# zju3dv/ENeRF

Hardware: AMD Instinct MI355X
Metric: rendered frames/sec @512x640 3-src-view (higher is better)
Workload: dtype f32

## Files before the change

### enerf_amd/csrc/capi.hip

```cpp
#include <stdarg.h>
#include <stdint.h>
#include <stdio.h>
#include <string.h>

#include "kernels.h"
#include "prep_job.h"

using namespace enerf;

namespace enerf {
__global__ __launch_bounds__(256) void k_zero(unsigned* __restrict__ p, long long n) {
    for (long long i = (long long)blockIdx.x * blockDim.x + threadIdx.x; i < n; i += (long long)gridDim.x * blockDim.x) p[i] = 0u;
}
void zero_async(void* p, size_t bytes, hipStream_t st) {
    const long long n = (long long)(bytes / 4);
    if (n <= 0) return;
    long long blocks = cdivl(n, 256 * 4);
    if (blocks > 4096) blocks = 4096;
    ENERF_LAUNCH_SIMPLE(k_zero, (unsigned)blocks, 256, 0, st, (unsigned*)p, n);
}
void zero_async2(void* p, size_t bytes_p, void* q, size_t bytes_q, hipStream_t st) {
    if ((char*)p + bytes_p == (char*)q && bytes_p % 4 == 0) { zero_async(p, bytes_p + bytes_q, st); return; }
    zero_async(p, bytes_p, st);
    zero_async(q, bytes_q, st);
// ... 194 lines not shown
        if (im.pk8 >= 0) launch_conv3d_pk8_pack(w, wd, s.cin, p + im.pk8, st);
        if (im.b4 >= 0) launch_conv3d_b4_pack(w, wd, s.cin, p + im.b4, st);
        p += im.floats;
    }
    return check_launch("cost_reg_pack");
}
size_t enerf_cost_reg_workspace_bytes(int full, int B, int D, int h, int w) {
    long long floats[kNumBufs], f = 0;
    const int n = costreg_buffers(full, (long long)B * D * h * w, floats);
    for (int i = 0; i < n; ++i) f += floats[i];
    return (size_t)f * sizeof(float);
}
int enerf_cost_reg(const float* packed, int in_channels, int full, const float* vol, int B, int D, int h, int w,
                   float* feat, float* prob, void* workspace, size_t workspace_bytes, const enerf_options_t* options,
                   enerf_stream_t stream) {
    return cost_reg_run(packed, in_channels, full, vol, 0, B, D, h, w, feat, prob, workspace, workspace_bytes, options,
                        (hipStream_t)stream);
}
}
namespace enerf {
bool cost_reg_conv0_planar(const enerf_options_t& o, int in_channels, int full, int B, int D, int h, int w) {
    return cost_reg_plan(in_channels, full, B, D, h, w, o, device_cu_count()).vol_planar_ok;
}
int cost_reg_run(const float* packed, int in_channels, int full, const float* vol, int vol_planar, int B, int D, int h, int w,
                 float* feat, float* prob, void* workspace, size_t workspace_bytes, const enerf_options_t* options,
                 hipStream_t st, const CostRegHook* hook) {
    REQUIRE(packed && vol && feat && prob && workspace, "cost_reg: null pointer");
    REQUIRE(in_channels == 8 || in_channels == 16 || in_channels == 32, "cost_reg: in_channels=%d unsupported (8/16/32)",
            in_channels);
    REQUIRE(B > 0 && D > 0 && h > 0 && w > 0, "cost_reg: bad shape");
    int div = full ? 8 : 4;
    REQUIRE(D % div == 0 && h % div == 0 && w % div == 0, "cost_reg: D,h,w (%d,%d,%d) must be divisible by %d", D, h, w, div);
    if (workspace_bytes < enerf_cost_reg_workspace_bytes(full, B, D, h, w))
        return fail(ENERF_EWORKSPACE, "cost_reg: workspace too small");
    const CostRegPlan P = cost_reg_plan(in_channels, full, B, D, h, w, resolve_options(options), device_cu_count());
    if (vol_planar && !P.vol_planar_ok)
        return fail(ENERF_EINVAL, "cost_reg: a quad-planar volume needs the asynchronously staged conv0 kernel (conv3d_b4 0/2, D % 4 == 0, >= conv3d_lds_min_voxels)");
    float* buf[kNumBufs] = {};
    long long floats[kNumBufs];
    const int nbuf = costreg_buffers(full, (long long)B * D * h * w, floats);
    float* ws = (float*)workspace;
    for (int i = 0; i < nbuf; ++i) { buf[i] = ws; ws += floats[i]; }
    bool ok = true;
    const float* p = packed;
    for (int i = 0; i < P.n; ++i) {
        const LayerSpec& s = P.spec[i];
        const Conv3dImage im = layer_image(s);
        Conv3dDesc d = conv3d_desc(p, im, s.cin, s.cout, s.kind, s.relu);
        p += im.floats;
        d.in_planar = i == 0 ? vol_planar : (i == P.n - 1 && P.heads_planar);
// ... 624 lines not shown
```

### enerf_amd/csrc/conv3d.hip

```cpp

#include "kernels.h"

namespace enerf {

__host__ __device__ __forceinline__ void convt_axis(int par, int idx, int& k, int& dq) {
    if (par == 0) { k = 1; dq = 0; }
    else if (idx == 0) { k = 0; dq = 1; }
    else { k = 2; dq = 0; }
}
__host__ __device__ __forceinline__ int convt_class_ntaps(int cls) {
    return (1 + ((cls >> 2) & 1)) * (1 + ((cls >> 1) & 1)) * (1 + (cls & 1));
}
__host__ __device__ __forceinline__ int convt_class_offset(int cls) {
    int o = 0;
    for (int c = 0; c < cls; ++c) o += convt_class_ntaps(c);
    return o;
}

__host__ __device__ __forceinline__ int conv_cpl(int cin) { return cin >= 16 ? 4 : cin / 4; }

long long conv3d_packed_floats(int cin, int cout, int kind) {
    (void)kind;
    int rt = cdiv(cout, 16);
    return 27LL * (cin / 4) * rt * 64;
// ... 591 lines not shown
                   o.conv3d_lds_min_voxels > 0 ? o.conv3d_lds_min_voxels : 16384, vox_in, n_out, cdiv(L.cout, 16)};
    Conv3dRoute r;
    if ((r = route_t2_all(g)).family) return r;
    if ((r = route_t2_lds(g)).family) return r;
    if ((r = route_s2_lds(g)).family) return r;
    if ((r = route_b4(g)).family) return r;
    if ((r = route_pk8(g)).family) return r;
    if ((r = route_s1_lds(g)).family) return r;
    bool small;
    const Conv3dRoute global = route_global(g, &small);
    if ((r = route_wl(g, global, small)).family) return r;
    return global;
}
bool conv3d_route_planar_in(const Conv3dRoute& r) { return r.family == kRouteB4g || r.family == kRouteB4c; }
bool conv3d_route_planar_out(const Conv3dRoute& r) { return r.family == kRouteT2All && r.cout == 8; }
void conv3d_route_name(const Conv3dRoute& r, char* buf, size_t cap) {
    const char* tf = r.heads ? "true" : "false";
    switch (r.family) {
        case kRouteT2All: snprintf(buf, cap, "t2_all<%d,%d,%d,%d>", r.cin, r.cout, r.bd, r.bh); break;
        case kRouteT2Lds: snprintf(buf, cap, "t2_lds<%d>", r.cin); break;
        case kRouteS2Lds: snprintf(buf, cap, "s2_lds<%d>", r.cin); break;
        case kRouteB4: snprintf(buf, cap, "s1_b4<%d,%d,%s>", r.cin, r.bd, tf); break;
        case kRouteB4g: snprintf(buf, cap, "s1_b4g<%d,%d,%s>", r.cin, r.bd, tf); break;
        case kRouteB4c: snprintf(buf, cap, "s1_b4c<%d,%d,%s>", r.cin, r.bd, tf); break;
        case kRoutePk8: snprintf(buf, cap, "s1_pk8<%d,%d>", r.cin, r.bd); break;
        case kRouteS1Lds: snprintf(buf, cap, "s1_lds<%d,%d,%d,%d>", r.cin, r.rt, r.bd, r.bh); break;
        case kRouteWl: snprintf(buf, cap, "wl<%d,%d,%d>", r.cin, r.kind, r.ctb); break;
        case kRouteGlobal: snprintf(buf, cap, "conv3d<%d,%d,%d,%d,%d>", r.cin, r.rt, r.kind, r.ct, r.split); break;
        default: snprintf(buf, cap, "none"); break;
    }
// ... 69 lines not shown
```

### enerf_amd/csrc/conv3d_b4.hip

```cpp
#include "kernels.h"

namespace enerf {

#define ENERF_MFMA4(a, b, c) __builtin_amdgcn_mfma_f32_4x4x1f32((a), (b), (c), 0, 0, 0)

constexpr int kB4cRegs = 14;
long long conv3d_b4_packed_floats(int cin) { return 27LL * (cin / 4) * 48 + (long long)(cin / 4) * kB4cRegs * 64; }

__global__ __launch_bounds__(256) void k_conv3d_b4_pack(const float* __restrict__ w, const float* __restrict__ wd, int cin,
                                                        float* __restrict__ packed) {
    const long long total = 27LL * (cin / 4) * 48;
    const long long idx = (long long)blockIdx.x * blockDim.x + threadIdx.x;
    if (idx >= total) {
        const long long k = idx - total;
        if (k >= (long long)(cin / 4) * kB4cRegs * 64) return;
        const int l = (int)(k & 63), rr = (int)((k >> 6) % kB4cRegs), cq = (int)((k >> 6) / kB4cRegs), c = rr * 16 + (l >> 2);
        const int half = c & 1, ch = (c >> 1) & 3, tap = c >> 3;
        packed[idx] = tap < 27 ? w[((long long)(4 * half + (l & 3)) * cin + 4 * cq + ch) * 27 + tap] : 0.f;
        return;
    }
    const int e = (int)(idx % 48), r = e & 3, i = (e >> 2) & 3, slot = e >> 4;
    const long long q = idx / 48;
    const int nq = cin / 4, cq = (int)(q % nq), tap = (int)(q / nq);
    if (slot < 2) packed[idx] = w[((long long)(4 * slot + i) * cin + 4 * cq + r) * 27 + tap];
// ... 29 lines not shown
    int t = (int)xcd_contiguous(blockIdx.x, gridDim.x);
    const int bw = t % nbw; t /= nbw;
    const int bh = t % nbh; t /= nbh;
    const int bd = t % nbd;
    const int b = t / nbd;
    const int x0 = bw * BW, y0 = bh * BH, z0 = bd * BD;

    f32x4 acc[V][2];
    float dacc[V];
#pragma unroll
    for (int v = 0; v < V; ++v) { acc[v][0] = f32x4{0.f, 0.f, 0.f, 0.f}; acc[v][1] = f32x4{0.f, 0.f, 0.f, 0.f}; dacc[v] = 0.f; }
    const float* inb = in + (long long)b * D * H * W * CIN;
    const float* lbase = lds + ((zl * HY + yl) * HX + xl) * 4;
    const float* wbase = wlds + li * 4;

#pragma unroll 1
    for (int cb = 0; cb < NCB; ++cb) {
        if (cb > 0) __syncthreads();
        {
            constexpr int RW = HX * QV, SLOTS = 256 / RW, NR = HZ * HY, NITR = (NR + SLOTS - 1) / SLOTS;
            const int sub = tid % RW, slot = tid / RW, sdx = sub / QV, sq = sub - sdx * QV;
            const int gx = x0 + sdx - 1;
            const bool colok = slot < SLOTS && gx >= 0 && gx < W;
            float4 sv[NITR], wq[NWIT];
            bool sk[NITR];
            const float* src = inb + cb * CB + sq * 4;
#pragma unroll
            for (int it = 0; it < NITR; ++it) {
                const int r = slot + it * SLOTS, dz = r / HY, dy = r - dz * HY;
                const int gy = y0 + dy - 1, gz = z0 + dz - 1;
// ... 47 lines not shown
            if (HEADS) {
#pragma unroll
                for (int q = 0; q < QV; ++q)
#pragma unroll
                    for (int v = 0; v < V; ++v) {
                        const float4 bb = bq[tap & 1][v][q], wd = aq[tap & 1][q][NS - 1];
                        dacc[v] = __builtin_fmaf(wd.x, bb.x, dacc[v]);
                        dacc[v] = __builtin_fmaf(wd.y, bb.y, dacc[v]);
                        dacc[v] = __builtin_fmaf(wd.z, bb.z, dacc[v]);
                        dacc[v] = __builtin_fmaf(wd.w, bb.w, dacc[v]);
                        ENERF_PIN_VGPR(dacc[v]);
                    }
            }
#pragma unroll
            for (int q = 0; q < QV; ++q) {
                const float4 A0 = aq[tap & 1][q][0], A1 = aq[tap & 1][q][1];
                const float a0[4] = {A0.x, A0.y, A0.z, A0.w}, a1[4] = {A1.x, A1.y, A1.z, A1.w};
#pragma unroll
                for (int r = 0; r < 4; ++r)
#pragma unroll
                    for (int v = 0; v < V; ++v) {
                        const float4 bb = bq[tap & 1][v][q];
                        const float bx = r == 0 ? bb.x : r == 1 ? bb.y : r == 2 ? bb.z : bb.w;
                        acc[v][0] = ENERF_MFMA4(a0[r], bx, acc[v][0]);
                        acc[v][1] = ENERF_MFMA4(a1[r], bx, acc[v][1]);
                    }
            }
            __builtin_amdgcn_sched_barrier(0);
        }
    }

    const int x = x0 + xl, y = y0 + yl;
    if (x >= W || y >= H) return;
#pragma unroll
    for (int v = 0; v < V; ++v) {
        const int z = z0 + zl + 2 * v;
        if (z >= D) continue;
        const long long o = (((long long)b * D + z) * H + y) * W + x;
#pragma unroll
        for (int half = 0; half < 2; ++half) {
            float yv[4];
#pragma unroll
            for (int r = 0; r < 4; ++r) {
                yv[r] = acc[v][half][r] * scale[4 * half + r] + shift[4 * half + r];
                if (relu) yv[r] = fmaxf(yv[r], 0.f);
            }
            *reinterpret_cast<float4*>(out + o * 8 + 4 * half) = make_float4(yv[0], yv[1], yv[2], yv[3]);
        }
        if (HEADS && out2 != nullptr) out2[o] = dacc[v] * scale[8] + shift[8];
    }
}

__device__ float g_b4_zeros[64];

template <int CIN, int BD, bool HEADS>
__global__ __launch_bounds__(256, 3) void k_conv3d_s1_b4g(const float* __restrict__ wb4, const float* __restrict__ scale,
                                                          const float* __restrict__ shift, const float* __restrict__ in,
                                                          float* __restrict__ out, float* __restrict__ out2, int relu, int B,
                                                          int D, int H, int W, int nbd, int nbh, int nbw, int in_planar) {
    constexpr int BH = 8, BW = 16, V = BD / 2;
    constexpr int NQ = CIN / 4, NS = HEADS ? 3 : 2;
    constexpr int HX = BW + 2, HY = BH + 2, HZ = BD + 2, NVOX = HZ * HY * HX;
    constexpr int NCH = (NVOX + 63) / 64, PLANE = NCH * 64 * 4;
    constexpr int NW4 = 27 * NS * 4, NWCH = (NW4 + 63) / 64;
    constexpr int BUF = PLANE + NWCH * 64 * 4;
    constexpr int MYCH = (NCH + 3) / 4, MYW = (NWCH + 3) / 4;
    ENERF_DYN_SMEM(float, lds);

    const int tid = threadIdx.x, li = tid & 3, lane = tid & 63;
    const int wv = __builtin_amdgcn_readfirstlane(tid >> 6);
    const int m = lane & 31;
    const bool g1 = (m >= 4 && m < 12) || (m >= 16 && m < 20) || m >= 28;
    const int xl = g1 ? (m < 12 ? m - 4 : m < 20 ? m - 8 : m - 16) : (m < 4 ? m : m < 16 ? m - 8 : m - 12);
    const int yl = 4 * (wv & 1) + 2 * (lane >> 5) + (g1 ? 1 : 0), zl = wv >> 1;
// ... 104 lines not shown
            for (int r = 0; r < 4; ++r) {
                yv[r] = acc[v][half][r] * scale[4 * half + r] + shift[4 * half + r];
                if (relu) yv[r] = fmaxf(yv[r], 0.f);
            }
            *reinterpret_cast<float4*>(out + o * 8 + 4 * half) = make_float4(yv[0], yv[1], yv[2], yv[3]);
        }
        if (HEADS && out2 != nullptr) out2[o] = dacc[v] * scale[8] + shift[8];
    }
}

template <int CIN, int BD, bool HEADS>
__global__ __launch_bounds__(256, 3) void k_conv3d_s1_b4c(const float* __restrict__ wb4, const float* __restrict__ scale,
                                                          const float* __restrict__ shift, const float* __restrict__ in,
                                                          float* __restrict__ out, float* __restrict__ out2, int relu, int B,
                                                          int D, int H, int W, int nbd, int nbh, int nbw, int in_planar) {
    constexpr int BH = 8, BW = 16, V = BD / 2;
    constexpr int NQ = CIN / 4;
    constexpr int HX = BW + 2, HY = BH + 2, HZ = BD + 2, NVOX = HZ * HY * HX;
    constexpr int NCH = (NVOX + 63) / 64, PLANE = NCH * 64 * 4;
    constexpr int BUF = PLANE + (HEADS ? 256 : 0);
    constexpr int MYCH = (NCH + 3) / 4;
    static_assert(NQ % 2 == 0, "passes are processed in pairs (two register sets)");
    ENERF_DYN_SMEM(float, lds);

    const int tid = threadIdx.x, lane = tid & 63;
    const int wv = __builtin_amdgcn_readfirstlane(tid >> 6);
    const int m = lane & 31;
    const bool g1 = (m >= 4 && m < 12) || (m >= 16 && m < 20) || m >= 28;
    const int xl = g1 ? (m < 12 ? m - 4 : m < 20 ? m - 8 : m - 16) : (m < 4 ? m : m < 16 ? m - 8 : m - 12);
    const int yl = 4 * (wv & 1) + 2 * (lane >> 5) + (g1 ? 1 : 0), zl = wv >> 1;
// ... 162 lines not shown
```

### enerf_amd/csrc/frame.hip

```cpp
#include <stdint.h>
#include <string.h>

#include "kernels.h"
#include "prep_job.h"
#include "side_lane.h"

using namespace enerf;

namespace enerf {

constexpr int kMaskPerThread = 4;
constexpr int kMaskPerBlock = 256 * kMaskPerThread;

__device__ __forceinline__ bool mask_set(const unsigned char* m, int eb, long long i, long long n) {
    if (i >= n) return false;
    if (eb == 1) return m[i] != 0;
    const unsigned char* p = m + i * eb;
    unsigned v = 0;
    for (int k = 0; k < eb; ++k) v |= p[k];
    return v != 0;
}
__device__ __forceinline__ int block_exclusive_scan(int v, int* sh, int& total) {
    const int t = threadIdx.x;
    sh[t] = v;
// ... 129 lines not shown
}
int check_render_feat(const char* who, const enerf_cascade_t& c, int i, const FeatDims& fd, int Hr, int Wr, bool same_extent) {
    const int fl = c.render_im_feat_level[i];
    REQUIRE(fl >= 0 && fl <= 2 && fd.c[fl] == c.nerf_model_feat_ch[i],
            "%s: render_im_feat_level[%d]=%d does not have nerf_model_feat_ch=%d channels", who, i, fl, c.nerf_model_feat_ch[i]);
    if (same_extent)
        REQUIRE(fd.h[fl] == Hr && fd.w[fl] == Wr, "%s: level %d renders at %dx%d but feature level_%d is %dx%d "
                "(the HIP FeatureNet path needs render_scale == im_ibr_scale)", who, i, Hr, Wr, fl, fd.h[fl], fd.w[fl]);
    return ENERF_OK;
}

struct LevelPlan {
    int D, h, w, C, Hs, Ws;
    int Hr, Wr, render, masked, F, Ns;
    int fl, from_l2;
    long long n_rays;
    size_t proj, dv, nf, vol, feat3d, prob, depth, std, dmvs, tex, rays;
};
struct FramePlan {
    int tex2, hip_feats, cached;
    size_t f[3], featnet_ws, featnet_ws_bytes, costreg_ws, costreg_ws_bytes;
    size_t cam_exts, cam_ixts;
    size_t ray_index, ray_count, mask_ws;
    LevelPlan L[ENERF_MAX_LEVELS];
    size_t total_floats;
};

int make_plan(const enerf_frame_args_t* a, FramePlan* P, bool cached = false) {
    REQUIRE(a, "forward: null args");
    const enerf_cascade_t& c = a->cas;
// ... 27 lines not shown
        L.D = c.volume_planes[i];
        L.h = scaled(a->H, c.volume_scale[i]);
        L.w = scaled(a->W, c.volume_scale[i]);
        REQUIRE(i < 3, "forward: level %d has no feature map (FeatureNet has three scales)", i);
        L.C = fd.c[i]; L.Hs = fd.h[i]; L.Ws = fd.w[i];
        REQUIRE(!(i == 2 && P->tex2), "forward: level_2 texels cannot feed a cost volume");
        REQUIRE(L.D > 0 && L.h > 0 && L.w > 0, "forward: level %d volume is empty", i);
        if (i > 0) REQUIRE(c.depth_inv[i - 1], "forward: cascade levels after a depth-space level are undefined in the "
                                               "reference (utils.py:130)");
        REQUIRE(a->cost_reg_packed[i], "forward: cost_reg_packed[%d] missing", i);
        const long long nv = (long long)a->B * L.D * L.h * L.w;
        L.proj = take((size_t)a->B * a->S * 12);
        L.dv = take((size_t)nv);
        L.nf = take((size_t)a->B * 2 * L.h * L.w);
        L.vol = take((size_t)nv * L.C);
        L.feat3d = take((size_t)nv * 8);
        L.prob = take((size_t)nv);
        L.depth = take((size_t)a->B * L.h * L.w);
        L.std = take((size_t)a->B * L.h * L.w);
        L.dmvs = take((size_t)a->B * L.h * L.w);
        const size_t cw = enerf_cost_reg_workspace_bytes(i != 0, a->B, L.D, L.h, L.w);
        if (cw > P->costreg_ws_bytes) P->costreg_ws_bytes = cw;
        L.render = c.render_if[i] != 0;
        if (!L.render) continue;
        L.Hr = scaled(a->H, c.render_scale[i]);
        L.Wr = scaled(a->W, c.render_scale[i]);
        L.Ns = c.num_samples[i];
        L.F = c.nerf_model_feat_ch[i] + 3;
        REQUIRE(L.Hr > 1 && L.Wr > 1, "forward: level %d render extent too small", i);
        REQUIRE(a->nerf_packed[i], "forward: nerf_packed[%d] missing", i);
        REQUIRE(a->rgb[i] && a->depth[i] && a->weights[i] && a->depth_mvs[i] && a->std[i], "forward: level %d output missing", i);
// ... 287 lines not shown
            launch_feature_volume(f[i], proj, dv, a->B, a->S, L.C, L.Hs, L.Ws, L.D, L.h, L.w, vol, st, 1);
            rc = check_launch("build_feature_volume");
        }
        if (rc == ENERF_OK) mark(ENERF_STAGE_LEVEL(i, ENERF_STAGE_VOLUME));
        return rc;
    }

    int level_cost_reg(int i) {
        const LevelPlan& L = P.L[i];
        const CostRegHook hook = {[](void* self) { static_cast<FrameRun*>(self)->enqueue_stage2(); }, this, gate_mode == 4 ? 2 : 0};
        const CostRegHook* hk = nullptr;
        const bool gated_here = !stage2_enqueued && i == cas().num - 1;
        if (gated_here) {
            if (gate_mode == 3) enqueue_stage2(); else hk = &hook;
        }
        int rc = cost_reg_run(a->cost_reg_packed[i], L.C, i != 0, ws + L.vol, vol_planar, a->B, L.D, L.h, L.w, ws + L.feat3d, ws + L.prob,
                              ws + P.costreg_ws, P.costreg_ws_bytes, a->options, st, hk);
        if (gated_here) enqueue_stage2();
        if (rc == ENERF_OK && stage2_rc != ENERF_OK) rc = stage2_rc;
        if (rc == ENERF_OK) mark(ENERF_STAGE_LEVEL(i, ENERF_STAGE_COST_REG));
        return rc;
    }

    int level_depth(int i) {
        const enerf_cascade_t& c = cas();
        const LevelPlan& L = P.L[i];
        float *prob = ws + L.prob, *dv = ws + L.dv, *depth = ws + L.depth, *std = std_of(i);
        const bool defer_regression = !L.render && i + 1 < c.num && !(a->options && a->options->fuse_depth_prep == 1);
        if (defer_regression) { pending_prob = prob; pending_dv = dv; pending_D = L.D; pending_inv = c.depth_inv[i]; }
        else launch_depth_regression(prob, dv, a->B, L.D, L.h, L.w, c.depth_inv[i], depth, std, L.render ? a->depth_mvs[i] : nullptr, st);
        mark(ENERF_STAGE_LEVEL(i, ENERF_STAGE_DEPTH_REG));
        pdepth = depth; pstd = std; pnf = ws + L.nf; hp = L.h; wp = L.w;
// ... 695 lines not shown
```

### enerf_amd/csrc/kernels.h

```cpp
#pragma once
#include "common.h"
#include "../../include/enerf_hip.h"

namespace enerf {

using Options = enerf_options_t;
inline Options resolve_options(const enerf_options_t* o) { return o ? *o : Options{}; }
int fail(int code, const char* fmt, ...);
int check_launch(const char* what);
const char* last_error();
#define REQUIRE(cond, ...) \
    do { if (!(cond)) return ::enerf::fail(ENERF_EINVAL, __VA_ARGS__); } while (0)
int device_cu_count();
void zero_async(void* p, size_t bytes, hipStream_t st);
void zero_async2(void* p, size_t bytes_p, void* q, size_t bytes_q, hipStream_t st);

void launch_channels_last(const float* src, float* dst, int n, int C, long long P, int Cpad, hipStream_t st);
void launch_channels_first(const float* src, float* dst, int n, int C, long long P, int Cpad, hipStream_t st);
void launch_pack_img_feat_rgb(const float* im_feat, int C, int Hf, int Wf, const float* src_inps, int H, int W,
                              int Hr, int Wr, int tex, int n_img, float* out, hipStream_t st);
void launch_proj_mats(const float* src_ixts, const float* src_exts, const float* tar_ixt, const float* tar_ext, int B,
                      int S, float src_scale, float tar_scale, float* proj, hipStream_t st);
void launch_depth_values(const float* near_far, const float* pdepth, const float* pstd, const float* pnf, int B, int D,
                         int h, int w, int hp, int wp, int depth_inv, float* dv, float* nf_out, hipStream_t st);
// ... 1 lines not shown
                       float src_scale, float tar_scale, float* proj, const float* near_far, const float* pdepth,
                       const float* pstd, const float* pnf, int B, int D, int h, int w, int hp, int wp, int depth_inv,
                       float* dv, float* nf_out, hipStream_t st);
void launch_depth_regression(const float* prob, const float* dv, int B, int D, int h, int w, int depth_inv,
                             float* depth, float* std, float* depth_mvs, hipStream_t st);
bool launch_regress_and_values(const float* src_ixts, const float* src_exts, const float* tar_ixt, const float* tar_ext, int S,
                               float src_scale, float tar_scale, float* proj, const float* prob_p, const float* dv_p,
                               const float* nf_p, int Dp, int hp, int wp, int depth_inv_p, float* depth_p, float* std_p, int B,
                               int D, int h, int w, int depth_inv, float* dv, float* nf_out, hipStream_t st);
void launch_build_rays(const float* rays8, const float* depth, const float* std, const float* nf, int B, int N, int h,
                       int w, int Hr, int Wr, int depth_inv, float* rays12, hipStream_t st);

void launch_feature_volume(const float* feat_nhwc, const float* proj, const float* dv, int B, int S, int C, int Hs,
                           int Ws, int D, int h, int w, float* vol, hipStream_t st, int planar = 0);
bool cost_reg_conv0_planar(const enerf_options_t& o, int in_channels, int full, int B, int D, int h, int w);
struct CostRegHook { void (*fn)(void* ctx); void* ctx; int after_layer; };
int cost_reg_run(const float* packed, int in_channels, int full, const float* vol, int vol_planar, int B, int D, int h, int w,
                 float* feat, float* prob, void* workspace, size_t workspace_bytes, const enerf_options_t* options, hipStream_t st,
                 const CostRegHook* hook = nullptr);

enum ConvKind { kConvS1 = 0, kConvS2 = 1, kConvT2 = 2 };
struct Conv3dDesc {
    const float* w;
    const float* scale;
    const float* shift;
    int cin, cout, kind, relu;
    const float* w_pk8;
    const float* w_b4;
    const float* w_t2pair;
    int in_planar;
// ... 20 lines not shown
    kRouteGlobal
};
struct Conv3dRoute {
    int family = kRouteNone;
    int cin = 0, cout = 0, kind = 0;
    int bd = 0, bh = 0;
    bool heads = false;
    int rt = 0, ct = 0, split = 0;
    int ctb = 0, kdlo = 0, nkd = 0;
};
struct Conv3dLayer { int cin, cout, kind; bool pk8, b4, t2pair; };
Conv3dRoute conv3d_route(const Conv3dLayer& L, bool has_residual, bool has_out2, int B, int Di, int Hi, int Wi, const Options& o,
                         int cu_count);
bool conv3d_route_planar_in(const Conv3dRoute& r);
bool conv3d_route_planar_out(const Conv3dRoute& r);
void conv3d_route_name(const Conv3dRoute& r, char* buf, size_t cap);

void launch_conv3d_b4(const Conv3dDesc& L, const Conv3dRoute& r, const float* in, float* out, float* out2, int B, int D, int H, int W,
                      hipStream_t st);
void launch_conv3d_pk8(const Conv3dDesc& L, const Conv3dRoute& r, const float* in, float* out, float* out2, int B, int D, int H, int W,
                       hipStream_t st);
void launch_conv3d_s2_lds(const Conv3dDesc& L, const float* in, float* out, int B, int Di, int Hi, int Wi, hipStream_t st);
void launch_conv3d_t2_lds(const Conv3dDesc& L, const float* in, const float* residual, float* out, int B, int Di, int Hi, int Wi,
                          hipStream_t st);
void launch_conv3d_t2_all(const Conv3dDesc& L, const Conv3dRoute& r, const float* in, const float* residual, float* out, int B, int Di,
                          int Hi, int Wi, hipStream_t st);
bool launch_conv3d_wl(const Conv3dDesc& L, const Conv3dRoute& r, const float* in, float* out, int B, int Di, int Hi, int Wi,
                      hipStream_t st);
long long conv3d_packed_floats(int cin, int cout, int kind);
void launch_conv3d_pack(const float* w, const float* w2, int cout1, const float* bn_w, const float* bn_b, const float* bn_mean, const float* bn_var,
// ... 134 lines not shown
```

### enerf_amd/lib.py

```python
from __future__ import annotations

import contextlib
import ctypes as C
import os
import threading
from typing import Optional

import torch

_PKG = os.path.dirname(os.path.abspath(__file__))
LIB_PATH = os.path.join(_PKG, "libenerf_hip.so")
ABI_VERSION = 11

_f = C.c_void_p
_i = C.c_int
_ll = C.c_longlong
_fl = C.c_float


class ConvBn(C.Structure):
    _fields_ = [("w", _f), ("bn_weight", _f), ("bn_bias", _f), ("bn_mean", _f), ("bn_var", _f)]


class CostRegRaw(C.Structure):
# ... 2 lines not shown

class FeatNetRaw(C.Structure):
    _fields_ = [("conv", ConvBn * 6)] + [(n, _f) for n in ("toplayer_w", "toplayer_b", "lat1_w", "lat1_b", "lat0_w",
                                                            "lat0_b", "smooth1_w", "smooth1_b", "smooth0_w", "smooth0_b")]


class NerfRaw(C.Structure):
    _fields_ = [(n, _f) for n in ("view_w", "view_b", "glob_w", "glob_b", "aggw_w", "aggw_b", "fc_w", "fc_b",
                                  "lr0_w", "lr0_b", "sigma_w", "sigma_b", "col0_w", "col0_b", "col2_w", "col2_b")]


class Options(C.Structure):
    _fields_ = [("conv3d_global_only", _i), ("conv3d_lds_min_voxels", _ll), ("conv3d_pk8", _i),
                ("featnet_unfused", _i), ("featnet_smooth0_plain", _i), ("conv3d_b4", _i), ("single_stream", _i),
                ("side_gate", _i), ("fuse_depth_prep", _i), ("conv3d_t2_variant", _i), ("conv3d_small_variant", _i),
                ("render_precision", _i)]

    def __repr__(self):
        return "Options(" + ", ".join(f"{n}={getattr(self, n)}" for n, _ in self._fields_ if getattr(self, n)) + ")"


def throughput_options() -> "Options":
    return Options(single_stream=1)


def _opt(o):
    return None if o is None else C.byref(o)


class MlpBwdArgs(C.Structure):
    _fields_ = ([(n, _f) for n in ("vox", "x", "g_raw", "packed", "bimg", "g_vox", "g_x")] + [("save", C.c_void_p * 16),
# ... 142 lines not shown
    "enerf_pack_img_feat_rgb": (_i, [_f, _i, _i, _i, _f, _i, _i, _i, _i, _i, _i, _f, _f]),
    "enerf_feature_net_packed_floats": (_ll, []),
    "enerf_feature_net_pack": (_i, [C.POINTER(FeatNetRaw), _f, _f]),
    "enerf_feature_net_workspace_bytes": (C.c_size_t, [_i, _i, _i]),
    "enerf_feature_net": (_i, [_f, _f, _i, _i, _i, _f, _f, _f, _i, _f, C.c_size_t, C.POINTER(Options), _f]),
    "enerf_feature_net_stage": (_i, [_f, _f, _i, _i, _i, _f, _f, _f, _i, _f, C.c_size_t, _i, C.POINTER(Options), _f]),
    "enerf_pack_texels_cl": (_i, [_f, _i, _f, _i, _i, _i, _i, _i, _i, _f, _f]),
    "enerf_get_proj_mats": (_i, [_f, _f, _f, _f, _i, _i, _fl, _fl, _f, _f]),
    "enerf_get_depth_values": (_i, [_f, _f, _f, _f, _i, _i, _i, _i, _i, _i, _i, _f, _f, _f]),
    "enerf_level_prep": (_i, [_f, _f, _f, _f, _i, _i, _fl, _fl, _f, _f, _f, _f, _f, _i, _i, _i, _i, _i, _i, _f, _f, _f]),
    "enerf_build_feature_volume": (_i, [_f, _f, _f, _i, _i, _i, _i, _i, _i, _i, _i, _f, _f]),
    "enerf_cost_reg_packed_floats": (_ll, [_i, _i]),
    "enerf_cost_reg_pack": (_i, [C.POINTER(CostRegRaw), _f, _f]),
    "enerf_cost_reg_workspace_bytes": (C.c_size_t, [_i, _i, _i, _i, _i]),
    "enerf_cost_reg": (_i, [_f, _i, _i, _f, _i, _i, _i, _i, _f, _f, _f, C.c_size_t, C.POINTER(Options), _f]),
    "enerf_depth_regression": (_i, [_f, _f, _i, _i, _i, _i, _i, _f, _f, _f]),
    "enerf_build_rays": (_i, [_f, _f, _f, _f, _i, _i, _i, _i, _i, _i, _i, _f, _f]),
    "enerf_nerf_packed_floats": (_ll, [_i]),
    "enerf_nerf_pack": (_i, [C.POINTER(NerfRaw), _i, _i, _f, _f]),
    "enerf_render_rays": (_i, [C.POINTER(RenderArgs), _f]),
    "enerf_mask_compact_workspace_bytes": (C.c_size_t, [_ll]),
    "enerf_mask_compact": (_i, [C.c_void_p, _i, _ll, C.c_void_p, C.c_void_p, C.c_void_p, C.c_size_t, _f]),
    "enerf_forward_workspace_bytes": (C.c_size_t, [C.POINTER(FrameArgs)]),
    "enerf_forward": (_i, [C.POINTER(FrameArgs), _f]),
    "enerf_build_feature_volume_bwd": (_i, [_f, _f, _f, _f, _i, _i, _i, _i, _i, _i, _i, _i, _f, _f, _f]),
    "enerf_depth_regression_bwd": (_i, [_f, _f, _f, _f, _i, _i, _i, _i, _i, _f, _f, _f]),
    "enerf_conv_wgrad_workspace_bytes": (C.c_size_t, [_ll, _i, _i, _i, _i, _i]),
    "enerf_conv_wgrad": (_i, [_f, _f] + [_i] * 16 + [_f, C.c_void_p, C.c_size_t, _f]),
    "enerf_gemm_wgrad_workspace_bytes": (C.c_size_t, [_ll, _i, _i, _i]),
    "enerf_nerf_mlp_bwd": (_i, [C.POINTER(MlpBwdArgs), _f]),
# ... 304 lines not shown
        self._check(self.dll.enerf_cost_reg_pack(C.byref(raw), _ptr(packed), self.stream_of(packed)), "cost_reg_pack")
        return packed

    def cost_reg(self, packed, in_channels, full, vol, workspace=None, options=None, out=None):
        B, D, h, w, _ = vol.shape
        need = self.dll.enerf_cost_reg_workspace_bytes(int(full), B, D, h, w)
        if workspace is None or workspace.numel() * 4 < need:
            workspace = torch.empty(((need + 3) // 4,), dtype=torch.float32, device=vol.device)
        feat = _out(None if out is None else out[0], (B, D, h, w, 8), vol.device, "cost_reg")
        prob = _out(None if out is None else out[1], (B, D, h, w), vol.device, "cost_reg")
        self._check(self.dll.enerf_cost_reg(_ptr(packed), in_channels, int(full), _ptr(vol), B, D, h, w, _ptr(feat),
                                            _ptr(prob), _ptr(workspace), workspace.numel() * 4, _opt(options),
                                            self.stream_of(vol)), "cost_reg")
        return feat, prob

    def depth_regression(self, prob, dv, depth_inv, out=None):
        B, D, h, w = prob.shape
        depth = _out(None if out is None else out[0], (B, h, w), prob.device, "depth_regression")
        std = _out(None if out is None else out[1], (B, h, w), prob.device, "depth_regression")
        self._check(self.dll.enerf_depth_regression(_ptr(prob), _ptr(dv), B, D, h, w, int(depth_inv), _ptr(depth),
                                                    _ptr(std), self.stream_of(prob)), "depth_regression")
        return depth, std

    def build_rays(self, rays8, depth, std, near_far, Hr, Wr, depth_inv):
        B, N = rays8.shape[:2]
        h, w = depth.shape[-2:]
        out = torch.empty((B, N, 12), dtype=torch.float32, device=rays8.device)
        self._check(self.dll.enerf_build_rays(_ptr(rays8), _ptr(depth), _ptr(std), _ptr(near_far), B, N, h, w, Hr, Wr,
                                              int(depth_inv), _ptr(out), self.stream_of(out)), "build_rays")
        return out
# ... 1066 lines not shown
```

### include/enerf_hip.h

```cpp
#ifndef ENERF_HIP_H_
#define ENERF_HIP_H_

#include <stddef.h>

#ifdef __cplusplus
extern "C" {
#endif

#define ENERF_ABI_VERSION 11
#define ENERF_OK 0
#define ENERF_EINVAL (-1)
#define ENERF_ELAUNCH (-2)
#define ENERF_EWORKSPACE (-3)

typedef void* enerf_stream_t;

int enerf_abi_version(void);
const char* enerf_last_error(void);

int enerf_selftest_checks(void);
int enerf_selftest_primitives(const float* table, int table_floats, float* scratch, int blocks, unsigned* mismatches, enerf_stream_t stream);

typedef struct {
    int conv3d_global_only;
    long long conv3d_lds_min_voxels;
    int conv3d_pk8;
    int featnet_unfused;
    int featnet_smooth0_plain;
    int conv3d_b4;
    int single_stream;
    int side_gate;
    int fuse_depth_prep;
    int conv3d_t2_variant;
    int conv3d_small_variant;
    int render_precision;
} enerf_options_t;

int enerf_channels_last(const float* src, float* dst, int n, int C, long long P, int Cpad, enerf_stream_t stream);
int enerf_channels_first(const float* src, float* dst, int n, int C, long long P, int Cpad, enerf_stream_t stream);

int enerf_pack_img_feat_rgb(const float* im_feat, int C, int Hf, int Wf, const float* src_inps, int H, int W,
                            int Hr, int Wr, int tex, int n_img, float* out, enerf_stream_t stream);

typedef struct {
    const float* w;
    const float* bn_weight;
    const float* bn_bias;
    const float* bn_mean;
    const float* bn_var;
} enerf_conv_bn_t;
// ... 34 lines not shown
                               int Hs, int Ws, int D, int h, int w, float* vol, enerf_stream_t stream);

typedef struct {
    enerf_conv_bn_t conv[12];
    const float* feat_conv_w;
    const float* depth_conv_w;
    int in_channels;
    int full;
} enerf_costreg_raw_t;
long long enerf_cost_reg_packed_floats(int in_channels, int full);
int enerf_cost_reg_pack(const enerf_costreg_raw_t* raw, float* packed, enerf_stream_t stream);
size_t enerf_cost_reg_workspace_bytes(int full, int B, int D, int h, int w);
int enerf_cost_reg(const float* packed, int in_channels, int full, const float* vol, int B, int D, int h, int w,
                   float* feat, float* prob, void* workspace, size_t workspace_bytes, const enerf_options_t* options,
                   enerf_stream_t stream);

int enerf_depth_regression(const float* prob, const float* depth_values, int B, int D, int h, int w, int depth_inv,
                           float* depth, float* std, enerf_stream_t stream);

int enerf_build_rays(const float* rays8, const float* depth, const float* std, const float* near_far, int B, int N,
                     int h, int w, int Hr, int Wr, int depth_inv, float* rays12, enerf_stream_t stream);

typedef struct {
    const float *view_w, *view_b;
    const float *glob_w, *glob_b;
    const float *aggw_w, *aggw_b;
    const float *fc_w, *fc_b;
    const float *lr0_w, *lr0_b;
    const float *sigma_w, *sigma_b;
    const float *col0_w, *col0_b;
// ... 395 lines not shown
```

Before: 1313.

## Skip feature-head output in cost regulation for non-rendered levels

Adds a prob-only path for the cost-regularization heads. When a level is not rendered, its 8-channel feature volume is no longer computed or allocated, and a dedicated depth-only kernel computes just the probability head. This removes the feature-head FMAs and stores on the coarse level. The cost is extra code paths, a new option field that changes the ABI struct, and an error returned when the selected route cannot skip the feature output.

Result: faster. 1335 (median of 6 runs) (+1.7%).

```diff
diff --git a/enerf_amd/csrc/capi.hip b/enerf_amd/csrc/capi.hip
--- a/enerf_amd/csrc/capi.hip
+++ b/enerf_amd/csrc/capi.hip
@@ -232,7 +232,13 @@
 int enerf_cost_reg(const float* packed, int in_channels, int full, const float* vol, int B, int D, int h, int w,
                    float* feat, float* prob, void* workspace, size_t workspace_bytes, const enerf_options_t* options,
                    enerf_stream_t stream) {
+    REQUIRE(feat, "cost_reg: null pointer");
     return cost_reg_run(packed, in_channels, full, vol, 0, B, D, h, w, feat, prob, workspace, workspace_bytes, options,
+                        (hipStream_t)stream);
+}
+int enerf_cost_reg_prob(const float* packed, int in_channels, int full, const float* vol, int B, int D, int h, int w, float* prob,
+                        void* workspace, size_t workspace_bytes, const enerf_options_t* options, enerf_stream_t stream) {
+    return cost_reg_run(packed, in_channels, full, vol, 0, B, D, h, w, nullptr, prob, workspace, workspace_bytes, options,
                         (hipStream_t)stream);
 }
 }
@@ -240,10 +246,14 @@
 bool cost_reg_conv0_planar(const enerf_options_t& o, int in_channels, int full, int B, int D, int h, int w) {
     return cost_reg_plan(in_channels, full, B, D, h, w, o, device_cu_count()).vol_planar_ok;
 }
+bool cost_reg_feat_optional(const enerf_options_t& o, int in_channels, int full, int B, int D, int h, int w) {
+    const CostRegPlan P = cost_reg_plan(in_channels, full, B, D, h, w, o, device_cu_count());
+    return conv3d_route_optional_out(P.route[P.n - 1]);
+}
 int cost_reg_run(const float* packed, int in_channels, int full, const float* vol, int vol_planar, int B, int D, int h, int w,
                  float* feat, float* prob, void* workspace, size_t workspace_bytes, const enerf_options_t* options,
                  hipStream_t st, const CostRegHook* hook) {
-    REQUIRE(packed && vol && feat && prob && workspace, "cost_reg: null pointer");
+    REQUIRE(packed && vol && prob && workspace, "cost_reg: null pointer");
     REQUIRE(in_channels == 8 || in_channels == 16 || in_channels == 32, "cost_reg: in_channels=%d unsupported (8/16/32)",
             in_channels);
     REQUIRE(B > 0 && D > 0 && h > 0 && w > 0, "cost_reg: bad shape");
@@ -252,6 +262,8 @@
     if (workspace_bytes < enerf_cost_reg_workspace_bytes(full, B, D, h, w))
         return fail(ENERF_EWORKSPACE, "cost_reg: workspace too small");
     const CostRegPlan P = cost_reg_plan(in_channels, full, B, D, h, w, resolve_options(options), device_cu_count());
+    if (feat == nullptr && !conv3d_route_optional_out(P.route[P.n - 1]))
+        return fail(ENERF_EINVAL, "cost_reg: the heads' kernel at this shape and these options cannot skip the feature output (needs the batched-4x4 heads, conv3d_b4 != 1)");
     if (vol_planar && !P.vol_planar_ok)
         return fail(ENERF_EINVAL, "cost_reg: a quad-planar volume needs the asynchronously staged conv0 kernel (conv3d_b4 0/2, D % 4 == 0, >= conv3d_lds_min_voxels)");
     float* buf[kNumBufs] = {};
diff --git a/enerf_amd/csrc/conv3d.hip b/enerf_amd/csrc/conv3d.hip
--- a/enerf_amd/csrc/conv3d.hip
+++ b/enerf_amd/csrc/conv3d.hip
@@ -629,6 +629,9 @@
 }
 bool conv3d_route_planar_in(const Conv3dRoute& r) { return r.family == kRouteB4g || r.family == kRouteB4c; }
 bool conv3d_route_planar_out(const Conv3dRoute& r) { return r.family == kRouteT2All && r.cout == 8; }
+bool conv3d_route_optional_out(const Conv3dRoute& r) {
+    return r.heads && (r.family == kRouteB4 || r.family == kRouteB4g || r.family == kRouteB4c);
+}
 void conv3d_route_name(const Conv3dRoute& r, char* buf, size_t cap) {
     const char* tf = r.heads ? "true" : "false";
     switch (r.family) {
diff --git a/enerf_amd/csrc/conv3d_b4.hip b/enerf_amd/csrc/conv3d_b4.hip
--- a/enerf_amd/csrc/conv3d_b4.hip
+++ b/enerf_amd/csrc/conv3d_b4.hip
@@ -67,6 +67,7 @@
     const float* lbase = lds + ((zl * HY + yl) * HX + xl) * 4;
     const float* wbase = wlds + li * 4;
 
+    const bool feat = !HEADS || out != nullptr;
 #pragma unroll 1
     for (int cb = 0; cb < NCB; ++cb) {
         if (cb > 0) __syncthreads();
@@ -144,6 +145,7 @@
             }
 #pragma unroll
             for (int q = 0; q < QV; ++q) {
+                if (!feat) break;
                 const float4 A0 = aq[tap & 1][q][0], A1 = aq[tap & 1][q][1];
                 const float a0[4] = {A0.x, A0.y, A0.z, A0.w}, a1[4] = {A1.x, A1.y, A1.z, A1.w};
 #pragma unroll
@@ -168,7 +170,7 @@
         if (z >= D) continue;
         const long long o = (((long long)b * D + z) * H + y) * W + x;
 #pragma unroll
-        for (int half = 0; half < 2; ++half) {
+        for (int half = 0; half < 2 && feat; ++half) {
             float yv[4];
 #pragma unroll
             for (int r = 0; r < 4; ++r) {
@@ -182,12 +184,99 @@
 }
 
 __device__ float g_b4_zeros[64];
+
+template <int CIN, int BD>
+__device__ __forceinline__ void conv3d_b4_depth_only(const float* __restrict__ wb4, const float* __restrict__ scale,
+                                                     const float* __restrict__ shift, const float* __restrict__ in,
+                                                     float* __restrict__ out2, int D, int H, int W, int nbd, int nbh, int nbw,
+                                                     int in_planar) {
+    constexpr int BH = 8, BW = 16, V = BD / 2;
+    constexpr int NQ = CIN / 4;
+    constexpr int HX = BW + 2, HY = BH + 2, HZ = BD + 2, NVOX = HZ * HY * HX;
+    constexpr int NCH = (NVOX + 63) / 64, PLANE = NCH * 64 * 4, BUF = PLANE + 256, MYCH = (NCH + 3) / 4;
+    ENERF_DYN_SMEM(float, lds);
+
+    const int tid = threadIdx.x, lane = tid & 63;
+    const int wv = __builtin_amdgcn_readfirstlane(tid >> 6);
+    const int m = lane & 31;
+    const bool g1 = (m >= 4 && m < 12) || (m >= 16 && m < 20) || m >= 28;
+    const int xl = g1 ? (m < 12 ? m - 4 : m < 20 ? m - 8 : m - 16) : (m < 4 ? m : m < 16 ? m - 8 : m - 12);
+    const int yl = 4 * (wv & 1) + 2 * (lane >> 5) + (g1 ? 1 : 0), zl = wv >> 1;
+    int t = (int)xcd_contiguous(blockIdx.x, gridDim.x);
+    const int bw = t % nbw; t /= nbw;
+    const int bh = t % nbh; t /= nbh;
+    const int bd = t % nbd;
+    const int b = t / nbd;
+    const int x0 = bw * BW, y0 = bh * BH, z0 = bd * BD;
+    const float* inb = in + (long long)b * D * H * W * CIN;
+    const long long vstride = in_planar ? 4 : CIN, qstride = in_planar ? (long long)D * H * W * 4 : 4;
+
+    long long src_off[MYCH];
+#pragma unroll
+    for (int k = 0; k < MYCH; ++k) {
+        const int v = (wv + 4 * k) * 64 + lane;
+        const int dz = v / (HY * HX), r2 = v - dz * (HY * HX), dy = r2 / HX, dx = r2 - dy * HX;
+        const int gx = x0 + dx - 1, gy = y0 + dy - 1, gz = z0 + dz - 1;
+        const bool ok = v < NVOX && gx >= 0 && gx < W && gy >= 0 && gy < H && gz >= 0 && gz < D;
+        src_off[k] = ok ? (((long long)gz * H + gy) * W + gx) * vstride : -1;
+    }
+    const int wd_off = ((lane < 27 ? lane : 26) * NQ * 3 + 2) * 16;
+    auto issue = [&](int cq, float* buf) {
+#pragma unroll
+        for (int k = 0; k < MYCH; ++k)
+            if (wv + 4 * k < NCH)
+                glds16(src_off[k] >= 0 ? inb + src_off[k] + cq * qstride : g_b4_zeros, buf + (wv + 4 * k) * 256, lane);
+        if (wv == (NCH & 3)) glds16(wb4 + wd_off + cq * 48, buf + PLANE, lane);
+    };
+
+    float dacc[V];
+#pragma unroll
+    for (int v = 0; v < V; ++v) dacc[v] = 0.f;
+    issue(0, lds);
+#pragma unroll 1
+    for (int cq = 0; cq < NQ; ++cq) {
+        float* buf = lds + (cq & 1) * BUF;
+        glds_wait_all();
+        block_barrier_raw();
+        if (cq + 1 < NQ) issue(cq + 1, lds + ((cq + 1) & 1) * BUF);
+        const float* lbase = buf + ((zl * HY + yl) * HX + xl) * 4;
+        const float* wdl = buf + PLANE;
+#pragma unroll
+        for (int tap = 0; tap < 27; ++tap) {
+            const int kd = tap / 9, kh = (tap / 3) % 3, kw = tap % 3;
+            const float4 wd = *reinterpret_cast<const float4*>(wdl + tap * 4);
+#pragma unroll
+            for (int v = 0; v < V; ++v) {
+                const float4 bb = *reinterpret_cast<const float4*>(lbase + (((2 * v + kd) * HY + kh) * HX + kw) * 4);
+                dacc[v] = __builtin_fmaf(wd.x, bb.x, dacc[v]);
+                dacc[v] = __builtin_fmaf(wd.y, bb.y, dacc[v]);
+                dacc[v] = __builtin_fmaf(wd.z, bb.z, dacc[v]);
+                dacc[v] = __builtin_fmaf(wd.w, bb.w, dacc[v]);
+            }
+        }
+    }
+
+    const int x = x0 + xl, y = y0 + yl;
+    if (x >= W || y >= H) return;
+#pragma unroll
+    for (int v = 0; v < V; ++v) {
+        const int z = z0 + zl + 2 * v;
+        if (z >= D) continue;
+        out2[(((long long)b * D + z) * H + y) * W + x] = dacc[v] * scale[8] + shift[8];
+    }
+}
 
 template <int CIN, int BD, bool HEADS>
 __global__ __launch_bounds__(256, 3) void k_conv3d_s1_b4g(const float* __restrict__ wb4, const float* __restrict__ scale,
                                                           const float* __restrict__ shift, const float* __restrict__ in,
                                                           float* __restrict__ out, float* __restrict__ out2, int relu, int B,
                                                           int D, int H, int W, int nbd, int nbh, int nbw, int in_planar) {
+    if constexpr (HEADS) {
+        if (out == nullptr) {
+            if (out2 != nullptr) conv3d_b4_depth_only<CIN, BD>(wb4, scale, shift, in, out2, D, H, W, nbd, nbh, nbw, in_planar);
+            return;
+        }
+    }
     constexpr int BH = 8, BW = 16, V = BD / 2;
     constexpr int NQ = CIN / 4, NS = HEADS ? 3 : 2;
     constexpr int HX = BW + 2, HY = BH + 2, HZ = BD + 2, NVOX = HZ * HY * HX;
@@ -322,6 +411,12 @@
                                                           const float* __restrict__ shift, const float* __restrict__ in,
                                                           float* __restrict__ out, float* __restrict__ out2, int relu, int B,
                                                           int D, int H, int W, int nbd, int nbh, int nbw, int in_planar) {
+    if constexpr (HEADS) {
+        if (out == nullptr) {
+            if (out2 != nullptr) conv3d_b4_depth_only<CIN, BD>(wb4, scale, shift, in, out2, D, H, W, nbd, nbh, nbw, in_planar);
+            return;
+        }
+    }
     constexpr int BH = 8, BW = 16, V = BD / 2;
     constexpr int NQ = CIN / 4;
     constexpr int HX = BW + 2, HY = BH + 2, HZ = BD + 2, NVOX = HZ * HY * HX;
diff --git a/enerf_amd/csrc/frame.hip b/enerf_amd/csrc/frame.hip
--- a/enerf_amd/csrc/frame.hip
+++ b/enerf_amd/csrc/frame.hip
@@ -167,6 +167,7 @@
     int D, h, w, C, Hs, Ws;
     int Hr, Wr, render, masked, F, Ns;
     int fl, from_l2;
+    int prob_only;
     long long n_rays;
     size_t proj, dv, nf, vol, feat3d, prob, depth, std, dmvs, tex, rays;
 };
@@ -224,7 +225,9 @@
         L.dv = take((size_t)nv);
         L.nf = take((size_t)a->B * 2 * L.h * L.w);
         L.vol = take((size_t)nv * L.C);
-        L.feat3d = take((size_t)nv * 8);
+        L.prob_only = !c.render_if[i] && !(a->options && a->options->heads_keep_feat) &&
+                      cost_reg_feat_optional(resolve_options(a->options), L.C, i != 0, a->B, L.D, L.h, L.w);
+        if (!L.prob_only) L.feat3d = take((size_t)nv * 8);
         L.prob = take((size_t)nv);
         L.depth = take((size_t)a->B * L.h * L.w);
         L.std = take((size_t)a->B * L.h * L.w);
@@ -542,8 +545,8 @@
         if (gated_here) {
             if (gate_mode == 3) enqueue_stage2(); else hk = &hook;
         }
-        int rc = cost_reg_run(a->cost_reg_packed[i], L.C, i != 0, ws + L.vol, vol_planar, a->B, L.D, L.h, L.w, ws + L.feat3d, ws + L.prob,
-                              ws + P.costreg_ws, P.costreg_ws_bytes, a->options, st, hk);
+        int rc = cost_reg_run(a->cost_reg_packed[i], L.C, i != 0, ws + L.vol, vol_planar, a->B, L.D, L.h, L.w,
+                              L.prob_only ? nullptr : ws + L.feat3d, ws + L.prob, ws + P.costreg_ws, P.costreg_ws_bytes, a->options, st, hk);
         if (gated_here) enqueue_stage2();
         if (rc == ENERF_OK && stage2_rc != ENERF_OK) rc = stage2_rc;
         if (rc == ENERF_OK) mark(ENERF_STAGE_LEVEL(i, ENERF_STAGE_COST_REG));
diff --git a/enerf_amd/csrc/kernels.h b/enerf_amd/csrc/kernels.h
--- a/enerf_amd/csrc/kernels.h
+++ b/enerf_amd/csrc/kernels.h
@@ -39,6 +39,7 @@
 void launch_feature_volume(const float* feat_nhwc, const float* proj, const float* dv, int B, int S, int C, int Hs,
                            int Ws, int D, int h, int w, float* vol, hipStream_t st, int planar = 0);
 bool cost_reg_conv0_planar(const enerf_options_t& o, int in_channels, int full, int B, int D, int h, int w);
+bool cost_reg_feat_optional(const enerf_options_t& o, int in_channels, int full, int B, int D, int h, int w);
 struct CostRegHook { void (*fn)(void* ctx); void* ctx; int after_layer; };
 int cost_reg_run(const float* packed, int in_channels, int full, const float* vol, int vol_planar, int B, int D, int h, int w,
                  float* feat, float* prob, void* workspace, size_t workspace_bytes, const enerf_options_t* options, hipStream_t st,
@@ -89,6 +90,7 @@
                          int cu_count);
 bool conv3d_route_planar_in(const Conv3dRoute& r);
 bool conv3d_route_planar_out(const Conv3dRoute& r);
+bool conv3d_route_optional_out(const Conv3dRoute& r);
 void conv3d_route_name(const Conv3dRoute& r, char* buf, size_t cap);
 
 void launch_conv3d_b4(const Conv3dDesc& L, const Conv3dRoute& r, const float* in, float* out, float* out2, int B, int D, int H, int W,
diff --git a/enerf_amd/lib.py b/enerf_amd/lib.py
--- a/enerf_amd/lib.py
+++ b/enerf_amd/lib.py
@@ -40,7 +40,7 @@
     _fields_ = [("conv3d_global_only", _i), ("conv3d_lds_min_voxels", _ll), ("conv3d_pk8", _i),
                 ("featnet_unfused", _i), ("featnet_smooth0_plain", _i), ("conv3d_b4", _i), ("single_stream", _i),
                 ("side_gate", _i), ("fuse_depth_prep", _i), ("conv3d_t2_variant", _i), ("conv3d_small_variant", _i),
-                ("render_precision", _i)]
+                ("render_precision", _i), ("heads_keep_feat", _i)]
 
     def __repr__(self):
         return "Options(" + ", ".join(f"{n}={getattr(self, n)}" for n, _ in self._fields_ if getattr(self, n)) + ")"
@@ -213,6 +213,7 @@
     "enerf_cost_reg_pack": (_i, [C.POINTER(CostRegRaw), _f, _f]),
     "enerf_cost_reg_workspace_bytes": (C.c_size_t, [_i, _i, _i, _i, _i]),
     "enerf_cost_reg": (_i, [_f, _i, _i, _f, _i, _i, _i, _i, _f, _f, _f, C.c_size_t, C.POINTER(Options), _f]),
+    "enerf_cost_reg_prob": (_i, [_f, _i, _i, _f, _i, _i, _i, _i, _f, _f, C.c_size_t, C.POINTER(Options), _f]),
     "enerf_depth_regression": (_i, [_f, _f, _i, _i, _i, _i, _i, _f, _f, _f]),
     "enerf_build_rays": (_i, [_f, _f, _f, _f, _i, _i, _i, _i, _i, _i, _i, _f, _f]),
     "enerf_nerf_packed_floats": (_ll, [_i]),
@@ -547,6 +548,17 @@
                                             self.stream_of(vol)), "cost_reg")
         return feat, prob
 
+    def cost_reg_prob(self, packed, in_channels, full, vol, workspace=None, options=None, out=None):
+        B, D, h, w, _ = vol.shape
+        need = self.dll.enerf_cost_reg_workspace_bytes(int(full), B, D, h, w)
+        if workspace is None or workspace.numel() * 4 < need:
+            workspace = torch.empty(((need + 3) // 4,), dtype=torch.float32, device=vol.device)
+        prob = _out(out, (B, D, h, w), vol.device, "cost_reg_prob")
+        self._check(self.dll.enerf_cost_reg_prob(_ptr(packed), in_channels, int(full), _ptr(vol), B, D, h, w, _ptr(prob),
+                                                 _ptr(workspace), workspace.numel() * 4, _opt(options), self.stream_of(vol)),
+                    "cost_reg_prob")
+        return prob
+
     def depth_regression(self, prob, dv, depth_inv, out=None):
         B, D, h, w = prob.shape
         depth = _out(None if out is None else out[0], (B, h, w), prob.device, "depth_regression")
diff --git a/include/enerf_hip.h b/include/enerf_hip.h
--- a/include/enerf_hip.h
+++ b/include/enerf_hip.h
@@ -34,6 +34,7 @@
     int conv3d_t2_variant;
     int conv3d_small_variant;
     int render_precision;
+    int heads_keep_feat;
 } enerf_options_t;
 
 int enerf_channels_last(const float* src, float* dst, int n, int C, long long P, int Cpad, enerf_stream_t stream);
@@ -98,6 +99,8 @@
 int enerf_cost_reg(const float* packed, int in_channels, int full, const float* vol, int B, int D, int h, int w,
                    float* feat, float* prob, void* workspace, size_t workspace_bytes, const enerf_options_t* options,
                    enerf_stream_t stream);
+int enerf_cost_reg_prob(const float* packed, int in_channels, int full, const float* vol, int B, int D, int h, int w, float* prob,
+                        void* workspace, size_t workspace_bytes, const enerf_options_t* options, enerf_stream_t stream);
 
 int enerf_depth_regression(const float* prob, const float* depth_values, int B, int D, int h, int w, int depth_inv,
                            float* depth, float* std, enerf_stream_t stream);
```
